# coolbutuseless/zstdlite

Measured on NVIDIA B200. Metric: decompress_GBps_uncompressed, higher is better.
Workload: dtype u8

## Files before the change

### zstdlite_b200/csrc/zl_dec_exec.cuh

```cuda
#pragma once
#include "zl_common.cuh"
#include "zl_dec_entropy.cuh"

#if defined(__CUDACC__)

#define ZL_FULL 0xFFFFFFFFu

ZL_D void zl_warp_copy(u8* dst, const u8* src, u32 n, u32 lane)
{
    if (n < 64) { for (u32 i = lane; i < n; i += 32) dst[i] = src[i]; return; }
    if (((((size_t)dst) ^ ((size_t)src)) & 15) == 0) {
        u32 head = (u32)((16 - (((size_t)dst) & 15)) & 15);
        if (lane < head) dst[lane] = src[lane];
        u32 body = (n - head) >> 4;
        const uint4* s4 = (const uint4*)(src + head);
        uint4* d4 = (uint4*)(dst + head);
        u32 i = lane;
        for (; i + 96 < body; i += 128) {
            const uint4 a = s4[i], b = s4[i + 32], c = s4[i + 64], e = s4[i + 96];
            d4[i] = a; d4[i + 32] = b; d4[i + 64] = c; d4[i + 96] = e;
        }
        for (; i < body; i += 32) d4[i] = s4[i];
        u32 done = head + (body << 4);
        for (u32 i = done + lane; i < n; i += 32) dst[i] = src[i];
        return;
    }
    const u32 head = (u32)((4 - (((size_t)dst) & 3)) & 3);
    if (lane < head) dst[lane] = src[lane];
    const u8* s = src + head;
    u32* d4 = (u32*)(dst + head);
    const u32 words = (n - head) >> 2;
    const u32 sh = (u32)(((size_t)s) & 3) * 8;
    const u32* s4 = (const u32*)(((size_t)s) & ~(size_t)3);
    if (sh == 0) for (u32 i = lane; i < words; i += 32) d4[i] = s4[i];
    else {
        u32 i = lane;
        for (; i + 96 < words; i += 128) {
            const u32 a0 = s4[i], a1 = s4[i + 1], b0 = s4[i + 32], b1 = s4[i + 33], c0 = s4[i + 64], c1 = s4[i + 65], e0 = s4[i + 96], e1 = s4[i + 97];
            d4[i] = __funnelshift_r(a0, a1, sh); d4[i + 32] = __funnelshift_r(b0, b1, sh); d4[i + 64] = __funnelshift_r(c0, c1, sh); d4[i + 96] = __funnelshift_r(e0, e1, sh);
        }
        for (; i < words; i += 32) d4[i] = __funnelshift_r(s4[i], s4[i + 1], sh);
    }
    const u32 done = head + (words << 2);
    if (done + lane < n) dst[done + lane] = src[done + lane];
}

ZL_D void zl_warp_fill(u8* dst, u32 byte, u32 n, u32 lane)
{
    u32 head = (u32)((4 - (((size_t)dst) & 3)) & 3);
    if (head > n) head = n;
    if (lane < head) dst[lane] = (u8)byte;
    u32 body = (n - head) >> 2;
    u32 w = byte * 0x01010101u;
    u32* d4 = (u32*)(dst + head);
    for (u32 i = lane; i < body; i += 32) d4[i] = w;
    u32 done = head + (body << 2);
    for (u32 i = done + lane; i < n; i += 32) dst[i] = (u8)byte;
}

#define ZL_REPT_ID 0x00020100u
ZL_D u32 zl_rept_compose(u32 A, u32 B)
{
    const u32 m = (B >> 7) & 0x00010101u;
    const u32 mm = m * 0xFFu;
    const u32 r = (B & 0x00030303u & ~mm) | (0x00060504u & mm);
    const u32 sel = (r & 0xFu) | ((r >> 4) & 0xF0u) | ((r >> 8) & 0xF00u) | 0x3000u;
    return __byte_perm(A, B, sel) & 0x00FFFFFFu;
}

ZL_D void zl_lane_record(u64 rec, bool valid, const u32* xtab, u32& ll, u32& ml, u32& ob)
{
    ll = 0; ml = 0; ob = 0;
    if (!valid) return;
    if (rec & ZL_REC_B) { ll = (u32)rec & 0xFFFFu; ml = ((u32)rec >> 16) & 0xFFFFu; ob = (u32)(rec >> 32) & 0x7FFFFFFFu; return; }
    const u32 snap = (u32)rec, c = (u32)(rec >> 32);
    const u32 llCode = c & 63u, mlCode = (c >> 6) & 63u, aOF = (c >> 12) & 31u;
    const u32 xl = xtab[llCode], xm = xtab[36 + mlCode];
    const u32 aLL = xl >> 24, aML = xm >> 24;
    ob = (1u << aOF) + zl_shr(snap, 32u - aOF);
    ml = (xm & 0xFFFFFFu) + zl_shr(zl_shl(snap, aOF), 32u - aML);
    ll = (xl & 0xFFFFFFu) + zl_shr(zl_shl(snap, aOF + aML), 32u - aLL);
}
ZL_D u32 zl_rep_idx(u32 ll, u32 ml, u32 ob) { return (ml != 0 && ob >= 1 && ob <= 3) ? ob - 1 + (ll == 0 ? 1u : 0u) : 0u; }
ZL_D u32 zl_rept_of(bool isNew, u32 idx, u32 tag)
{
    if (isNew) return 0x00010000u | 0x80u | tag;
    if (idx == 1) return 0x00020001u;
    if (idx == 2) return 0x00010002u;
    return ZL_REPT_ID;
}
ZL_D u32 zl_rept_scan(u32 T, u32 lane)
{
#pragma unroll
    for (int d = 1; d < 32; d <<= 1) {
        const u32 A = __shfl_up_sync(ZL_FULL, T, d);
        if ((int)lane >= d) T = zl_rept_compose(A, T);
    }
    return T;
}
ZL_D u32 zl_batch_offsets(u32 ll, u32 ml, u32 ob, u32 lane, u32& h0, u32& h1, u32& h2)
{
    const bool isM = ml != 0, isNew = isM && ob >= 4;
    const u32 idx = zl_rep_idx(ll, ml, ob);
    u32 off;
    if (__ballot_sync(ZL_FULL, idx == 3)) {
        off = 0;
        u32 hh[3] = {h0, h1, h2};
        for (u32 l = 0; l < 32; l++) {
            const u32 lll = __shfl_sync(ZL_FULL, ll, l), lml = __shfl_sync(ZL_FULL, ml, l), lob = __shfl_sync(ZL_FULL, ob, l);
            const u32 o = zl_rep_resolve(hh, lll, lml, lob);
            if (l == lane) off = o;
        }
        h0 = hh[0]; h1 = hh[1]; h2 = hh[2];
        return off;
    }
    const u32 fresh = ob - 3;
    const u32 T = zl_rept_scan(zl_rept_of(isNew, idx, lane), lane);
    u32 E = __shfl_up_sync(ZL_FULL, T, 1);
    if (lane == 0) E = ZL_REPT_ID;
    const u32 eb = (E >> (8 * idx)) & 0xFFu;
    const u32 fromLane = __shfl_sync(ZL_FULL, fresh, eb & 31u);
    const u32 fromHist = (eb & 3u) == 0 ? h0 : ((eb & 3u) == 1 ? h1 : h2);
    off = isNew ? fresh : ((eb & 0x80u) ? fromLane : fromHist);
    const u32 Lt = __shfl_sync(ZL_FULL, T, 31);
    const u32 b0 = Lt & 0xFFu, b1 = (Lt >> 8) & 0xFFu, b2 = (Lt >> 16) & 0xFFu;
    const u32 f0 = __shfl_sync(ZL_FULL, fresh, b0 & 31u), f1 = __shfl_sync(ZL_FULL, fresh, b1 & 31u), f2 = __shfl_sync(ZL_FULL, fresh, b2 & 31u);
    const u32 n0 = (b0 & 0x80u) ? f0 : ((b0 & 3u) == 0 ? h0 : ((b0 & 3u) == 1 ? h1 : h2));
    const u32 n1 = (b1 & 0x80u) ? f1 : ((b1 & 3u) == 0 ? h0 : ((b1 & 3u) == 1 ? h1 : h2));
    const u32 n2 = (b2 & 0x80u) ? f2 : ((b2 & 3u) == 0 ? h0 : ((b2 & 3u) == 1 ? h1 : h2));
    h0 = n0; h1 = n1; h2 = n2;
    return off;
}
ZL_D void zl_batch_positions(u32 ll, u32 ml, u32 lane, u32& sl, u32& so, u32& totalL, u32& totalO)
{
    sl = ll; so = ll + ml;
#pragma unroll
    for (int d = 1; d < 32; d <<= 1) {
        u32 a = __shfl_up_sync(ZL_FULL, sl, d), b = __shfl_up_sync(ZL_FULL, so, d);
        if ((int)lane >= d) { sl += a; so += b; }
    }
    totalL = __shfl_sync(ZL_FULL, sl, 31); totalO = __shfl_sync(ZL_FULL, so, 31);
}
ZL_D u32 zl_flat_owner(u32 rs, u32 j)
{
    u32 k = 0;
#pragma unroll
    for (int st = 16; st >= 1; st >>= 1) {
        const u32 v = __shfl_sync(ZL_FULL, rs, (k + st - 1) & 31);
        if (v <= j) k += st;
    }
    return k & 31;
}

#define ZL_SEG_LIT 0x80000000u
#ifndef ZL_XB
#define ZL_XB 4
#endif
#define ZL_XBATCH (32 * ZL_XB)
#define ZL_XROWS (32 * ZL_XB)
struct ZlExecSm {
    uint4 seg[2 * ZL_XBATCH];
    union { u32 fresh[ZL_XBATCH]; uint2 row[ZL_XROWS]; } u;
};
ZL_D uint2 zl_lds64(u32 a) { uint2 v; asm volatile("ld.shared.v2.u32 {%0, %1}, [%2];" : "=r"(v.x), "=r"(v.y) : "r"(a)); return v; }
ZL_D uint4 zl_lds128(u32 a) { uint4 v; asm volatile("ld.shared.v4.u32 {%0, %1, %2, %3}, [%4];" : "=r"(v.x), "=r"(v.y), "=r"(v.z), "=r"(v.w) : "r"(a)); return v; }
ZL_D u32 zl_lds32s(u32 a) { u32 v; asm volatile("ld.shared.u32 %0, [%1];" : "=r"(v) : "r"(a)); return v; }
ZL_D u32 zl_mod_small(u32 k, u32 d, u32 rcpA)
{
    const u32 q = __umulhi(k, zl_lds32s(rcpA + (d << 2)));
    u32 r = k - q * d;
    if (r >= d) r -= d;
    return r;
}
ZL_D const u8* zl_ptr_add(u32 lo, u32 hi, u32 j) { return reinterpret_cast<const u8*>((((u64)hi << 32) | lo) + j); }

ZL_D void zl_batch_offsets4(const u32 (&ll)[ZL_XB], const u32 (&ml)[ZL_XB], const u32 (&ob)[ZL_XB], u32 lane, u32* fresh,
                            u32& h0, u32& h1, u32& h2, u32 (&off)[ZL_XB])
{
    u32 idx[ZL_XB], t[ZL_XB];
    bool minus1 = false;
#pragma unroll
    for (int m = 0; m < ZL_XB; m++) {
        idx[m] = zl_rep_idx(ll[m], ml[m], ob[m]);
        minus1 |= idx[m] == 3;
        t[m] = zl_rept_of(ml[m] != 0 && ob[m] >= 4, idx[m], ZL_XB * lane + (u32)m);
    }
    if (__any_sync(ZL_FULL, minus1)) {
        u32 hh[3] = {h0, h1, h2};
        for (u32 l = 0; l < 32; l++) {
#pragma unroll
            for (int m = 0; m < ZL_XB; m++) {
                const u32 lll = __shfl_sync(ZL_FULL, ll[m], l), lml = __shfl_sync(ZL_FULL, ml[m], l), lob = __shfl_sync(ZL_FULL, ob[m], l);
                const u32 o = zl_rep_resolve(hh, lll, lml, lob);
                if (l == lane) off[m] = o;
            }
        }
        h0 = hh[0]; h1 = hh[1]; h2 = hh[2];
        return;
    }
#if ZL_XB == 4
    *reinterpret_cast<uint4*>(fresh + 4u * lane) = make_uint4(ob[0] - 3u, ob[1] - 3u, ob[2] - 3u, ob[3] - 3u);
    const u32 t01 = zl_rept_compose(t[0], t[1]), t012 = zl_rept_compose(t01, t[2]);
    const u32 T = zl_rept_scan(zl_rept_compose(t012, t[3]), lane);
#else
    *reinterpret_cast<uint2*>(fresh + 2u * lane) = make_uint2(ob[0] - 3u, ob[1] - 3u);
    const u32 t01 = zl_rept_compose(t[0], t[1]);
    const u32 T = zl_rept_scan(t01, lane);
#endif
    u32 E = __shfl_up_sync(ZL_FULL, T, 1);
    if (lane == 0) E = ZL_REPT_ID;
    __syncwarp();
#if ZL_XB == 4
    const u32 e[ZL_XB] = {E, zl_rept_compose(E, t[0]), zl_rept_compose(E, t01), zl_rept_compose(E, t012)};
#else
    const u32 e[ZL_XB] = {E, zl_rept_compose(E, t[0])};
#endif
#pragma unroll
    for (int m = 0; m < ZL_XB; m++) {
        const u32 eb = (e[m] >> (8u * idx[m])) & 0xFFu;
        const u32 fromTag = fresh[eb & (ZL_XBATCH - 1)];
        const u32 fromHist = (eb & 3u) == 0 ? h0 : ((eb & 3u) == 1 ? h1 : h2);
        off[m] = (ml[m] != 0 && ob[m] >= 4) ? ob[m] - 3u : ((eb & 0x80u) ? fromTag : fromHist);
    }
    const u32 Lt = __shfl_sync(ZL_FULL, T, 31);
    const u32 b0 = Lt & 0xFFu, b1 = (Lt >> 8) & 0xFFu, b2 = (Lt >> 16) & 0xFFu;
    const u32 f0 = fresh[b0 & (ZL_XBATCH - 1)], f1 = fresh[b1 & (ZL_XBATCH - 1)], f2 = fresh[b2 & (ZL_XBATCH - 1)];
    const u32 n0 = (b0 & 0x80u) ? f0 : ((b0 & 3u) == 0 ? h0 : ((b0 & 3u) == 1 ? h1 : h2));
    const u32 n1 = (b1 & 0x80u) ? f1 : ((b1 & 3u) == 0 ? h0 : ((b1 & 3u) == 1 ? h1 : h2));
    const u32 n2 = (b2 & 0x80u) ? f2 : ((b2 & 3u) == 0 ? h0 : ((b2 & 3u) == 1 ? h1 : h2));
    h0 = n0; h1 = n1; h2 = n2;
}

template <bool kDict>
ZL_D u32 zl_exec_block(u8* out, u32 op, u32 cap, u32 capErr, const ZlBlockHdr& h, const u8* __restrict__ lit, u32 rleByte, u32 litMode,
                       const u64* __restrict__ recs, const u8* __restrict__ dict, u32 dictSize, u32 (&hist)[3], const u32* xtab, const u32* rcp,
                       ZlExecSm* sm, u32 lane, u32& regen)
{
    const u32 nrec = h.nrec, litSize = h.litSize;
    const u32 leMask = 0xFFFFFFFFu >> (31u - lane);
    const u32 segA = (u32)__cvta_generic_to_shared(sm->seg), rowA = (u32)__cvta_generic_to_shared(sm->u.row), rcpA = (u32)__cvta_generic_to_shared(rcp);
    const bool rleLits = litMode == 1;
    u32 outPos = op, litPos = 0;
    u32 h0 = hist[0], h1 = hist[1], h2 = hist[2];
    auto outPtr = [&](i32 sp) -> const u8* { return (kDict && sp < 0) ? dict + ((i32)dictSize + sp) : out + sp; };
    for (u32 base = 0; base < nrec; base += ZL_XBATCH) {
        const u32 i0 = base + ZL_XB * lane;
        ulonglong2 ra = make_ulonglong2(0ull, 0ull), rb = ra;
        if (i0 < nrec) ra = __ldcs(reinterpret_cast<const ulonglong2*>(recs + i0));
        if (ZL_XB == 4 && i0 + 2 < nrec) rb = __ldcs(reinterpret_cast<const ulonglong2*>(recs + i0 + 2));
        if (i0 + ZL_XBATCH < nrec) asm volatile("prefetch.global.L1 [%0];" ::"l"(recs + i0 + ZL_XBATCH));
        u32 ll[ZL_XB], ml[ZL_XB], ob[ZL_XB], off[ZL_XB];
        zl_lane_record(ra.x, i0 < nrec, xtab, ll[0], ml[0], ob[0]);
        zl_lane_record(ra.y, i0 + 1 < nrec, xtab, ll[1], ml[1], ob[1]);
#if ZL_XB == 4
        zl_lane_record(rb.x, i0 + 2 < nrec, xtab, ll[2], ml[2], ob[2]);
        zl_lane_record(rb.y, i0 + 3 < nrec, xtab, ll[3], ml[3], ob[3]);
#endif
        u32 L = 0, O = 0, nseg = 0;
#pragma unroll
        for (int m = 0; m < ZL_XB; m++) { L += ll[m]; O += ll[m] + ml[m]; nseg += (ll[m] ? 1u : 0u) + (ml[m] ? 1u : 0u); }
        u32 sl = L | (nseg << 23), so = O;
#pragma unroll
        for (int d = 1; d < 32; d <<= 1) {
            const u32 a = __shfl_up_sync(ZL_FULL, sl, d), b = __shfl_up_sync(ZL_FULL, so, d);
            if ((int)lane >= d) { sl += a; so += b; }
        }
        const u32 tot = __shfl_sync(ZL_FULL, sl, 31), totalO = __shfl_sync(ZL_FULL, so, 31);
        const u32 totalL = tot & 0x7FFFFFu;
        if (totalL > litSize - litPos) return ZL_E_corruption_detected;
        if ((outPos - op) + totalO > cap) return capErr;
        zl_batch_offsets4(ll, ml, ob, lane, sm->u.fresh, h0, h1, h2, off);
        const u32 ord0 = (sl >> 23) - nseg;
        u8* const ob8 = out + outPos;
        {
            u32 f = so - O, li = litPos + (sl & 0x7FFFFFu) - L, ord = ord0;
            bool bad = false;
#pragma unroll
            for (int m = 0; m < ZL_XB; m++) {
                if (ll[m]) { const u64 P = (u64)(size_t)lit + li - f; sm->seg[ord++] = make_uint4((u32)P, (u32)(P >> 32), f, ZL_SEG_LIT); }
                f += ll[m]; li += ll[m];
                bad |= ml[m] != 0 && (off[m] == 0 || off[m] > outPos + f + dictSize);
                if (ml[m]) { const u64 P = (u64)(size_t)ob8 - off[m]; sm->seg[ord++] = make_uint4((u32)P, (u32)(P >> 32), f, off[m]); }
                f += ml[m];
            }
            if (__any_sync(ZL_FULL, bad)) return ZL_E_corruption_detected;
        }
        const u32 mis = (u32)((size_t)ob8 & 31u);
        const u32 totalA = totalO + mis;
        u32 segsBefore = 0;
        for (u32 w0 = 0; w0 < totalA; w0 += ZL_XROWS * 32) {
            __syncwarp();
#if ZL_XB == 4
            reinterpret_cast<uint4*>(sm->u.row)[2 * lane] = make_uint4(0u, 0u, 0u, 0u);
            reinterpret_cast<uint4*>(sm->u.row)[2 * lane + 1] = make_uint4(0u, 0u, 0u, 0u);
#else
            reinterpret_cast<uint4*>(sm->u.row)[lane] = make_uint4(0u, 0u, 0u, 0u);
#endif
            __syncwarp();
#pragma unroll
            for (u32 k = 0; k < 2 * ZL_XB; k++) {
                const u32 a = zl_lds32s(segA + (((ord0 + k) & (2 * ZL_XBATCH - 1)) << 4) + 8u) + mis - w0;
                if (k < nseg && a < ZL_XROWS * 32) atomicOr(&sm->u.row[a >> 5].x, 1u << (a & 31u));
            }
            __syncwarp();
            {
#if ZL_XB == 4
                uint4 qa = zl_lds128(rowA + lane * 32u), qb = zl_lds128(rowA + lane * 32u + 16u);
                const u32 c0 = __popc(qa.x), c1 = __popc(qa.z), c2 = __popc(qb.x), c3 = __popc(qb.z);
#else
                uint4 qa = zl_lds128(rowA + lane * 16u);
                const u32 c0 = __popc(qa.x), c1 = __popc(qa.z), c2 = 0, c3 = 0;
#endif
                u32 inc = c0 + c1 + c2 + c3;
#pragma unroll
                for (int d = 1; d < 32; d <<= 1) { const u32 a = __shfl_up_sync(ZL_FULL, inc, d); if ((int)lane >= d) inc += a; }
                const u32 ex = segsBefore + inc - (c0 + c1 + c2 + c3);
                qa.y = ex; qa.w = ex + c0;
#if ZL_XB == 4
                qb.y = ex + c0 + c1; qb.w = ex + c0 + c1 + c2;
                reinterpret_cast<uint4*>(sm->u.row)[2 * lane] = qa;
                reinterpret_cast<uint4*>(sm->u.row)[2 * lane + 1] = qb;
#else
                reinterpret_cast<uint4*>(sm->u.row)[lane] = qa;
#endif
                segsBefore += __shfl_sync(ZL_FULL, inc, 31);
            }
            __syncwarp();
            const u32 wEnd = min(totalA, w0 + ZL_XROWS * 32);
            for (u32 a0 = w0; a0 < wEnd; a0 += 64) {
                const uint4 ri = zl_lds128(rowA + ((a0 - w0) >> 5) * 8u);
                const u32 ja = a0 + lane - mis, jb = ja + 32;
                const u32 d0 = a0 < mis ? lane - (mis - a0) : lane;
                if ((ri.x | ri.z) == 0u && a0 + 64 <= totalA) {
                    const uint4 s = zl_lds128(segA + (((ri.y - 1u) & (2 * ZL_XBATCH - 1)) << 4));
                    u32 va = rleByte, vb = rleByte;
                    if (s.w < 64u) {
                        u32 ta = ja - s.w, tb = jb - s.w;
                        if ((i32)ta >= (i32)s.z) ta = s.z - s.w + zl_mod_small(ja - s.z, s.w, rcpA);
                        if ((i32)tb >= (i32)s.z) tb = s.z - s.w + zl_mod_small(jb - s.z, s.w, rcpA);
                        va = *outPtr((i32)(outPos + ta)); vb = *outPtr((i32)(outPos + tb));
                    } else if (!(s.w == ZL_SEG_LIT && rleLits)) {
                        const u8* pa = zl_ptr_add(s.x, s.y, ja);
                        const u8* pb = zl_ptr_add(s.x, s.y, jb);
                        if (kDict && s.w != ZL_SEG_LIT) { pa = outPtr((i32)(outPos + ja - s.w)); pb = outPtr((i32)(outPos + jb - s.w)); }
                        va = *pa; vb = *pb;
                    }
                    ob8[ja] = (u8)va; ob8[jb] = (u8)vb;
                    __syncwarp();
                    continue;
                }
                const u32 c0 = ri.y + __popc(ri.x & leMask) - 1u, c1 = ri.w + __popc(ri.z & leMask) - 1u;
                const uint4 sa = zl_lds128(segA + ((c0 & (2 * ZL_XBATCH - 1)) << 4)), sb = zl_lds128(segA + ((c1 & (2 * ZL_XBATCH - 1)) << 4));
                const bool aa = ja < totalO, ab = jb < totalO;
                bool na = aa && sa.w <= d0, nb = ab && sb.w <= d0 + 32u;
                const u8* pa = zl_ptr_add(sa.x, sa.y, ja);
                const u8* pb = zl_ptr_add(sb.x, sb.y, jb);
                if (kDict) {
                    if (sa.w != ZL_SEG_LIT) pa = outPtr((i32)(outPos + ja - sa.w));
                    if (sb.w != ZL_SEG_LIT) pb = outPtr((i32)(outPos + jb - sb.w));
                }
                u32 va = rleByte, vb = rleByte;
                if (aa && !na && !(sa.w == ZL_SEG_LIT && rleLits)) va = *pa;
                if (ab && !nb && !(sb.w == ZL_SEG_LIT && rleLits)) vb = *pb;
                if (__any_sync(ZL_FULL, na || nb)) {
                    const u32 j0 = a0 < mis ? 0u : a0 - mis;
                    u32 ta = ja - sa.w, tb = jb - sb.w;
                    if (na && ta >= sa.z) { ta = sa.z - sa.w + zl_mod_small(ja - sa.z, sa.w, rcpA); if ((i32)ta < (i32)j0) { na = false; va = *outPtr((i32)(outPos + ta)); } }
                    if (nb && tb >= sb.z) { tb = sb.z - sb.w + zl_mod_small(jb - sb.z, sb.w, rcpA); if ((i32)tb < (i32)j0) { nb = false; vb = *outPtr((i32)(outPos + tb)); } }
                    const u32 ra_ = ta + mis - a0, rb_ = tb + mis - a0;
                    while (__any_sync(ZL_FULL, na || nb)) {
                        const u32 w = (va & 0xFFu) | (na ? 0u : 0x100u) | ((vb & 0xFFu) << 16) | (nb ? 0u : 0x1000000u);
                        const u32 wa = __shfl_sync(ZL_FULL, w, ra_ & 31u) >> ((ra_ & 32u) >> 1), wb = __shfl_sync(ZL_FULL, w, rb_ & 31u) >> ((rb_ & 32u) >> 1);
                        if (na && (wa & 0x100u)) { va = wa & 0xFFu; na = false; }
                        if (nb && (wb & 0x100u)) { vb = wb & 0xFFu; nb = false; }
                    }
                }
                if (aa) ob8[ja] = (u8)va;
                if (ab) ob8[jb] = (u8)vb;
                __syncwarp();
            }
        }
        outPos += totalO; litPos += totalL;
    }
    const u32 lastLL = litSize - litPos;
    if ((outPos - op) + lastLL > cap) return capErr;
    if (litMode == 1) zl_warp_fill(out + outPos, rleByte, lastLL, lane);
    else zl_warp_copy(out + outPos, lit + litPos, lastLL, lane);
    hist[0] = h0; hist[1] = h1; hist[2] = h2;
    regen = outPos - op + lastLL;
    return 0;
}

#define ZL_P1 0x9E3779B185EBCA87ULL
#define ZL_P2 0xC2B2AE3D27D4EB4FULL
#define ZL_P3 0x165667B19E3779F9ULL
#define ZL_P4 0x85EBCA77C2B2AE63ULL
#define ZL_P5 0x27D4EB2F165667C5ULL
ZL_D u64 zl_rotl64(u64 x, int r) { return (x << r) | (x >> (64 - r)); }
ZL_D u64 zl_xround(u64 acc, u64 in) { return zl_rotl64(acc + in * ZL_P2, 31) * ZL_P1; }
ZL_D u64 zl_xmerge(u64 h, u64 v) { return (h ^ zl_xround(0, v)) * ZL_P1 + ZL_P4; }
ZL_D u64 zl_ld64u(const u8* p)
{
    if ((((size_t)p) & 7) == 0) return *(const u64*)p;
    if ((((size_t)p) & 3) == 0) return (u64)(*(const u32*)p) | ((u64)(*(const u32*)(p + 4)) << 32);
    return zl_rd64(p);
}
ZL_D u64 zl_xxh_seed(u32 q) { return q == 0 ? (ZL_P1 + ZL_P2) : (q == 1 ? ZL_P2 : (q == 2 ? 0ull : (0ull - ZL_P1))); }
ZL_D u64 zl_quad_xxh64_from(const u8* p, u32 len, u64 v, u32 s0, u32 q, u32 qmask, u32 qbase)
{
    u64 h;
    u32 done = 0;
    if (len >= 32) {
        const u32 stripes = len >> 5;
        const u8* pp = p + 8 * q;
        for (u32 s = s0; s < stripes; s++) v = zl_xround(v, zl_ld64u(pp + 32 * s));
        const u64 v1 = __shfl_sync(qmask, v, qbase + 0), v2 = __shfl_sync(qmask, v, qbase + 1);
        const u64 v3 = __shfl_sync(qmask, v, qbase + 2), v4 = __shfl_sync(qmask, v, qbase + 3);
        h = zl_rotl64(v1, 1) + zl_rotl64(v2, 7) + zl_rotl64(v3, 12) + zl_rotl64(v4, 18);
        h = zl_xmerge(h, v1); h = zl_xmerge(h, v2); h = zl_xmerge(h, v3); h = zl_xmerge(h, v4);
        done = stripes << 5;
    } else h = ZL_P5;
    h += (u64)len;
    const u8* t = p + done; u32 r = len - done;
    while (r >= 8) { h ^= zl_xround(0, zl_rd64(t)); h = zl_rotl64(h, 27) * ZL_P1 + ZL_P4; t += 8; r -= 8; }
    if (r >= 4) { h ^= (u64)zl_rd32(t) * ZL_P1; h = zl_rotl64(h, 23) * ZL_P2 + ZL_P3; t += 4; r -= 4; }
    while (r) { h ^= (u64)(*t++) * ZL_P5; h = zl_rotl64(h, 11) * ZL_P1; r--; }
    h ^= h >> 33; h *= ZL_P2; h ^= h >> 29; h *= ZL_P3; h ^= h >> 32;
    return h;
}
ZL_D u64 zl_quad_xxh64(const u8* p, u32 len, u32 q, u32 qmask, u32 qbase) { return zl_quad_xxh64_from(p, len, zl_xxh_seed(q), 0, q, qmask, qbase); }

#define ZL_XXH_CHUNK 2048u
ZL_D u64 zl_warp_xxh64(const u8* p, u32 len, u8 (*buf)[ZL_XXH_CHUNK], u32 lane)
{
    const u32 nchunks = len / ZL_XXH_CHUNK;
    u64 v = zl_xxh_seed(lane & 3);
    if (nchunks) {
        uint4 r[4];
#pragma unroll
        for (int i = 0; i < 4; i++) r[i] = __ldg((const uint4*)p + i * 32 + lane);
        for (u32 c = 0; c < nchunks; c++) {
            uint4* b4 = (uint4*)buf[c & 1];
#pragma unroll
            for (int i = 0; i < 4; i++) b4[i * 32 + lane] = r[i];
            __syncwarp();
            if (c + 1 < nchunks) {
                const uint4* g = (const uint4*)(p + (size_t)(c + 1) * ZL_XXH_CHUNK);
#pragma unroll
                for (int i = 0; i < 4; i++) r[i] = __ldg(g + i * 32 + lane);
            }
            if (lane < 4) {
                const u64* b8 = (const u64*)buf[c & 1] + lane;
#pragma unroll 8
                for (u32 s = 0; s < ZL_XXH_CHUNK / 32; s++) v = zl_xround(v, b8[4 * s]);
            }
        }
        __syncwarp();
    }
    u64 h = 0;
    if (lane < 4) h = zl_quad_xxh64_from(p, len, v, nchunks * (ZL_XXH_CHUNK / 32), lane, 0xFu, 0);
    return __shfl_sync(ZL_FULL, h, 0);
}
#endif
```

### zstdlite_b200/csrc/zl_dec_kernels.cu

```cuda
#include "zl_dec_entropy.cuh"
#include "zl_dec_exec.cuh"
#include "zl_dec_large.cuh"
#include "zl_launch.h"
#include "zl_plan.h"
#include <mutex>
#include <stdlib.h>

__constant__ ZlConstTables c_tables = {
    ZL_LL_BASE_INIT, ZL_ML_BASE_INIT, ZL_LL_BITS_INIT, ZL_ML_BITS_INIT,
    ZL_LL_DEFNORM_INIT, ZL_ML_DEFNORM_INIT, ZL_OF_DEFNORM_INIT};

__global__ void __launch_bounds__(128)
zl_k_index(const ZlFrameDesc* __restrict__ descs, ZlFrameInfo* __restrict__ infos, ZlBlockHdr* hdrArena, ZlUnit* units, u32* unitCount,
           u32 unitCap, u32 nframes, u32 frameBase, const ZlDictDev* dict)
{
    const u32 i = blockIdx.x * blockDim.x + threadIdx.x;
    if (i >= nframes) return;
    const ZlFrameDesc d = descs[i];
    ZlFrameInfo info;
    zl_index_frame(d, info, hdrArena + d.hdrBase, frameBase + i, dict ? dict->dictID : 0u, (dict && dict->hasEntropy) ? 1u : 0u,
                   units, unitCount, unitCap);
    infos[i] = info;
}

__device__ __forceinline__ u32 zl_fetch_units(u32* cursor, u32 lane, u32 count = ZL_QUADS_PER_WARP)
{
    u32 base = 0;
    if (lane == 0) base = atomicAdd(cursor, count);
    return __shfl_sync(0xFFFFFFFFu, base, 0);
}

#ifndef ZL_LIT_RING
#define ZL_LIT_RING 1
#endif
__global__ void __launch_bounds__(32)
zl_k_literals(const ZlFrameDesc* __restrict__ descs, ZlFrameInfo* __restrict__ infos, const ZlBlockHdr* hdrArena,
              u8* litArena, const ZlUnit* __restrict__ units, const u32* __restrict__ unitCount, u32* cursor, const ZlDictDev* dict)
{
    extern __shared__ __align__(16) u8 smraw[];
    ZlLitSm* fs = reinterpret_cast<ZlLitSm*>(smraw);
    const u32 lane = threadIdx.x, quad = lane >> 2, q = lane & 3;
    const u32 qmask = 0xFu << (quad * 4);
    ZlLitSm& f = fs[quad];
    const u32 ring = ZL_LIT_RING ? zl_smem_addr(smraw + ZL_QUADS_PER_WARP * sizeof(ZlLitSm)) + lane * 16u : 0u;
    u16* dictHuf = reinterpret_cast<u16*>(smraw + ZL_QUADS_PER_WARP * sizeof(ZlLitSm) + (ZL_LIT_RING ? ZL_LIT_RING_SLOTS * 32 * 16 : 0));
    if (dict && dict->hasEntropy) {
        const uint4* g = reinterpret_cast<const uint4*>(dict->huf);
        for (u32 i = lane; i < 2048 * 2 / 16; i += 32) reinterpret_cast<uint4*>(dictHuf)[i] = g[i];
        __syncwarp();
    }
    const u32 nunits = *unitCount;
    for (;;) {
        const u32 ubase = zl_fetch_units(cursor, lane);
        if (ubase >= nunits) break;
        const u32 u = ubase + quad;
        if (u < nunits) {
            const ZlUnit un = units[u];
            const ZlFrameDesc d = descs[un.frame];
            const ZlBlockHdr* hdrs = hdrArena + d.hdrBase;
            const u32 litMode = (hdrs[un.block].flags >> 4) & 3;
            if (litMode == 2) {
                u8* lits = (hdrs[un.block].flags & ZL_BLK_DIRECT) ? d.dst + hdrs[un.block].outOff - hdrs[un.block].litOff : litArena + d.litBase;
                const u32 bias = (u32)(((size_t)d.src) & 3);
                const u32* wbase = reinterpret_cast<const u32*>(d.src - bias);
                u32 useDict = 0;
                if (q == 0) zl_lit_unit_head(f, d, hdrs, un.block, wbase, bias, &useDict);
                useDict = __shfl_sync(qmask, useDict, quad * 4);
                __syncwarp(qmask);
                const u32 fill = f.ctl.needHufFill, ns = f.ctl.err ? 0u : f.ctl.nStreams;
                if (useDict) { if (q == 0) f.ctl.hufLog = dict->hufLog; }
                else if (fill && !f.ctl.err) zl_huf_fill(f, q);
                __syncwarp(qmask);
                if (q < ns)
                    f.ctl.sErr[q] = zl_huf_stream(useDict ? dictHuf : f.huf, f.ctl.hufLog, wbase, bias, f.ctl.sBeg[q], f.ctl.sEnd[q],
                                                  lits + f.ctl.sOut[q], f.ctl.sLen[q], ring);
                __syncwarp(qmask);
                if (q == 0) { const u32 e = zl_lit_unit_finish(f); if (e) infos[un.frame].err = e; }
                __syncwarp(qmask);
            }
        }
        __syncwarp();
    }
}

#define ZL_XTAB_BYTES ((ZL_XTAB_WORDS * 4 + 15) & ~15)
#ifndef ZL_SEQ_RING
#define ZL_SEQ_RING 1
#endif
__global__ void __launch_bounds__(32)
zl_k_sequences(const ZlFrameDesc* __restrict__ descs, ZlFrameInfo* __restrict__ infos, ZlBlockHdr* hdrArena,
               u64* recArena, i16* normArena, const ZlUnit* __restrict__ units, const u32* __restrict__ unitCount, u32* cursor,
               const ZlDictDev* dict)
{
    extern __shared__ __align__(16) u8 smraw[];
    u32* xtab = reinterpret_cast<u32*>(smraw);
    ZlSeqSm* fs = reinterpret_cast<ZlSeqSm*>(smraw + ZL_XTAB_BYTES);
    const ZlConstTables& ct = c_tables;
    const u32 lane = threadIdx.x, quad = lane / ZL_SEQ_G, q = lane % ZL_SEQ_G;
    const u32 qmask = (0xFFFFFFFFu >> (32 - ZL_SEQ_G)) << (quad * ZL_SEQ_G);
    for (u32 i = lane; i < ZL_XTAB_WORDS; i += 32)
        xtab[i] = i < 36 ? (c_tables.llBase[i] | ((u32)c_tables.llBits[i] << 24)) : (c_tables.mlBase[i - 36] | ((u32)c_tables.mlBits[i - 36] << 24));
    __syncwarp();
    ZlSeqSm& f = fs[quad];
    const u32 ring = ZL_SEQ_RING ? zl_smem_addr(smraw + ZL_XTAB_BYTES + ZL_SEQ_UNITS * sizeof(ZlSeqSm)) + quad * 16u : 0u;
    i16* norm = normArena + ((size_t)blockIdx.x * ZL_SEQ_UNITS + quad) * (3 * ZL_NORM_STRIDE);
    const u32 nunits = *unitCount;
    const u32 take = (nunits <= 1024u && ZL_SEQ_UNITS > 8u) ? 8u : (u32)ZL_SEQ_UNITS;
    for (;;) {
        const u32 ubase = zl_fetch_units(cursor, lane, take);
        if (ubase >= nunits) break;
        const u32 u = ubase + quad;
        if (quad < take && u < nunits) {
            const ZlUnit un = units[u];
            const ZlFrameDesc d = descs[un.frame];
            ZlBlockHdr* hdrs = hdrArena + d.hdrBase;
            if (hdrs[un.block].nbSeq) {
                const u32 bias = (u32)(((size_t)d.src) & 3);
                const u32* wbase = reinterpret_cast<const u32*>(d.src - bias);
                if (q == 0) zl_seq_head(f, d, hdrs, un.block, ct, norm);
                __syncwarp(qmask);
                const u32 build = f.ctl.err ? 0u : f.ctl.needBuild, useDict = f.ctl.err ? 0u : f.ctl.useDict;
                if (useDict) {
                    if (useDict & 1) { for (u32 i = q; i < 512; i += ZL_SEQ_G) f.fseLL[i] = dict->fseLL[i]; if (q == 0) f.ctl.tlog[0] = dict->tlog[0]; }
                    if (useDict & 2) { for (u32 i = q; i < 256; i += ZL_SEQ_G) f.fseOF[i] = dict->fseOF[i]; if (q == 0) f.ctl.tlog[1] = dict->tlog[1]; }
                    if (useDict & 4) { for (u32 i = q; i < 512; i += ZL_SEQ_G) f.fseML[i] = dict->fseML[i]; if (q == 0) f.ctl.tlog[2] = dict->tlog[2]; }
                }
                if (build) {
#if ZL_SEQ_G >= 3
                    if (q < 3) zl_seq_fse_build(f, q, norm);
#elif ZL_SEQ_G == 2
                    if (q == 0) { zl_seq_fse_build(f, 0, norm); zl_seq_fse_build(f, 1, norm); } else zl_seq_fse_build(f, 2, norm);
#else
                    for (u32 t = 0; t < 3; t++) zl_seq_fse_build(f, t, norm);
#endif
                }
                __syncwarp(qmask);
                if (q == 0) {
                    const u32 nrec = zl_seq_decode(f, recArena + d.recBase + hdrs[un.block].recOff, wbase, bias, ct, xtab, ring);
                    hdrs[un.block].nrec = nrec;
                    if (f.ctl.err) infos[un.frame].err = f.ctl.err;
                }
                __syncwarp(qmask);
            }
        }
        __syncwarp();
    }
}

template <bool kDict>
__global__ void __launch_bounds__(ZL_EXEC_WARPS * 32, ZL_EXEC_MIN_CTAS)
zl_k_execute(const ZlFrameDesc* __restrict__ descs, ZlFrameInfo* __restrict__ infos,
             const ZlBlockHdr* __restrict__ hdrArena, const u64* __restrict__ recArena,
             const u8* __restrict__ litArena, u64* __restrict__ results, u32 nframes, const ZlDictDev* dict)
{
    __shared__ u32 xtab[ZL_XTAB_WORDS];
    __shared__ __align__(16) ZlExecSm execSm[ZL_EXEC_WARPS];
    __shared__ u32 rcp[64];
    for (u32 i = threadIdx.x; i < ZL_XTAB_WORDS; i += ZL_EXEC_WARPS * 32)
        xtab[i] = i < 36 ? (c_tables.llBase[i] | ((u32)c_tables.llBits[i] << 24)) : (c_tables.mlBase[i - 36] | ((u32)c_tables.mlBits[i - 36] << 24));
    if (threadIdx.x < 64) rcp[threadIdx.x] = threadIdx.x ? 0xFFFFFFFFu / threadIdx.x : 0u;
    __syncthreads();
    const u32 lane = threadIdx.x & 31;
    const u32 frame = blockIdx.x * ZL_EXEC_WARPS + (threadIdx.x >> 5);
    if (frame >= nframes) return;
    const ZlFrameInfo info = infos[frame];
    if (info.err) { if (lane == 0) results[frame] = (u64)0 - (u64)info.err; return; }
    const ZlFrameDesc d = descs[frame];
    if (d.large) return;
    const ZlBlockHdr* hdrs = hdrArena + d.hdrBase;
    const u8* dictContent = kDict ? dict->content : nullptr;
    const u32 dictSize = kDict ? dict->contentSize : 0u;
    u32 hist[3] = {1, 4, 8};
    if (kDict && dict->hasEntropy) { hist[0] = dict->rep[0]; hist[1] = dict->rep[1]; hist[2] = dict->rep[2]; }
    u32 op = 0, err = 0;
    for (u32 b = 0; b < info.nblocks && !err; b++) {
        const ZlBlockHdr h = hdrs[b];
        const u32 type = h.flags & 3;
        const u32 room = d.dstCap - op;
        if (type != 2) {
            if (h.regenSize > room) { err = ZL_E_dstSize_tooSmall; break; }
            if (type == 0) zl_warp_copy(d.dst + op, d.src + h.srcOff, h.regenSize, lane);
            else zl_warp_fill(d.dst + op, (h.flags >> 8) & 0xFF, h.regenSize, lane);
            op += h.regenSize;
        } else if (h.flags & ZL_BLK_DIRECT) {
            op += h.litSize;
        } else {
            const u32 litMode = (h.flags >> 4) & 3;
            const u8* lit = litMode == 0 ? d.src + h.srcOff : litArena + d.litBase + h.litOff;
            u32 cap = room, capErr = ZL_E_dstSize_tooSmall, regen = 0;
            if (cap > ZL_BLOCKSIZE_MAX) { cap = ZL_BLOCKSIZE_MAX; capErr = ZL_E_corruption_detected; }
            err = zl_exec_block<kDict>(d.dst, op, cap, capErr, h, lit, (h.flags >> 8) & 0xFF, litMode, recArena + d.recBase + h.recOff,
                                       dictContent, dictSize, hist, xtab, rcp, &execSm[threadIdx.x >> 5], lane, regen);
            op += regen;
        }
        __syncwarp();
    }
    if (!err && info.contentSize != ~0ull && info.contentSize != (u64)op) err = ZL_E_corruption_detected;
    if (lane == 0) {
        results[frame] = err ? (u64)0 - (u64)err : (u64)op;
        infos[frame].err = err; infos[frame].totalOut = op;
    }
}

#define ZL_L_WARPS 4
__device__ __forceinline__ void zl_fill_xtab(u32* xtab, u32 tid, u32 nthreads)
{
    for (u32 i = tid; i < ZL_XTAB_WORDS; i += nthreads)
        xtab[i] = i < 36 ? (c_tables.llBase[i] | ((u32)c_tables.llBits[i] << 24)) : (c_tables.mlBase[i - 36] | ((u32)c_tables.mlBits[i - 36] << 24));
}
__global__ void __launch_bounds__(ZL_L_WARPS * 32)
zl_k_lblock_scan(const u32* __restrict__ largeIdx, const ZlFrameDesc* __restrict__ descs, const ZlFrameInfo* __restrict__ infos,
                 const ZlBlockHdr* __restrict__ hdrArena, const u64* __restrict__ recArena, ZlLChunk* lcArena)
{
    __shared__ u32 xtab[ZL_XTAB_WORDS];
    zl_fill_xtab(xtab, threadIdx.x, ZL_L_WARPS * 32);
    __syncthreads();
    const u32 frame = largeIdx[blockIdx.y], c = blockIdx.z * ZL_L_WARPS + (threadIdx.x >> 5), lane = threadIdx.x & 31;
    const ZlFrameInfo info = infos[frame];
    if (info.err) return;
    const ZlFrameDesc d = descs[frame];
    ZlLChunk* lc = lcArena + ((d.recBase >> ZL_LCHUNK_LOG) + d.hdrBase);
    for (u32 b = blockIdx.x; b < info.nblocks; b += gridDim.x) {
        const ZlBlockHdr h = hdrArena[d.hdrBase + b];
        if ((h.flags & 3) != 2 || !h.nrec || c >= zl_lchunks(h.nrec)) continue;
        const u32 r0 = c << ZL_LCHUNK_LOG, r1 = min(h.nrec, r0 + ZL_LCHUNK_RECS);
        zl_lchunk_scan(recArena + d.recBase + h.recOff, r0, r1, xtab, lane, lc[zl_lchunk_index(h.recOff, b) + c]);
    }
}
__global__ void __launch_bounds__(128)
zl_k_lblock_compose(const u32* __restrict__ largeIdx, const ZlFrameDesc* __restrict__ descs, const ZlFrameInfo* __restrict__ infos,
                    const ZlBlockHdr* __restrict__ hdrArena, ZlLBlock* lbArena, ZlLChunk* lcArena, u32 spread)
{
    const u32 frame = largeIdx[blockIdx.y];
    const ZlFrameInfo info = infos[frame];
    if (info.err) return;
    const ZlFrameDesc d = descs[frame];
    ZlLChunk* lc = lcArena + ((d.recBase >> ZL_LCHUNK_LOG) + d.hdrBase);
    for (u32 b = blockIdx.x * 128 + threadIdx.x; b < info.nblocks; b += gridDim.x * 128) {
        const ZlBlockHdr h = hdrArena[d.hdrBase + b];
        ZlLChunk* C = lc + zl_lchunk_index(h.recOff, b);
        if (spread) zl_lblock_spread(h, lbArena[d.hdrBase + b], C);
        else zl_lblock_compose(h, C, lbArena[d.hdrBase + b]);
    }
}
__global__ void __launch_bounds__(32)
zl_k_lframe_prefix(const u32* __restrict__ largeIdx, const ZlFrameDesc* __restrict__ descs, ZlFrameInfo* __restrict__ infos,
                   const ZlBlockHdr* __restrict__ hdrArena, ZlLBlock* lbArena, const ZlDictDev* dict)
{
    const u32 frame = largeIdx[blockIdx.x];
    if (threadIdx.x != 0) return;
    const ZlFrameInfo info = infos[frame];
    if (info.err) return;
    const ZlFrameDesc d = descs[frame];
    u32 r0 = 1, r1 = 4, r2 = 8, total = 0;
    if (dict && dict->hasEntropy) { r0 = dict->rep[0]; r1 = dict->rep[1]; r2 = dict->rep[2]; }
    const u32 err = zl_lframe_prefix(d, info, hdrArena + d.hdrBase, lbArena + d.hdrBase, r0, r1, r2, &total);
    infos[frame].err = err; infos[frame].totalOut = total;
}
template <bool kDict>
__global__ void __launch_bounds__(ZL_L_WARPS * 32)
zl_k_lblock_emit(const u32* __restrict__ largeIdx, const ZlFrameDesc* __restrict__ descs, ZlFrameInfo* __restrict__ infos,
                 const ZlBlockHdr* __restrict__ hdrArena, const u64* __restrict__ recArena, const u8* __restrict__ litArena,
                 const ZlLBlock* __restrict__ lbArena, const ZlLChunk* __restrict__ lcArena, u32* parentArena, const ZlDictDev* dict)
{
    __shared__ u32 xtab[ZL_XTAB_WORDS];
    zl_fill_xtab(xtab, threadIdx.x, ZL_L_WARPS * 32);
    __syncthreads();
    const u32 frame = largeIdx[blockIdx.y], c = blockIdx.z * ZL_L_WARPS + (threadIdx.x >> 5), lane = threadIdx.x & 31;
    const ZlFrameInfo info = infos[frame];
    if (info.err) return;
    const ZlFrameDesc d = descs[frame];
    const ZlLChunk* lc = lcArena + ((d.recBase >> ZL_LCHUNK_LOG) + d.hdrBase);
    for (u32 b = blockIdx.x; b < info.nblocks; b += gridDim.x) {
        const ZlBlockHdr h = hdrArena[d.hdrBase + b];
        const bool comp = (h.flags & 3) == 2;
        const u32 nch = comp ? zl_lchunks(h.nrec) : 1u;
        if (c >= nch) continue;
        const u32 litMode = (h.flags >> 4) & 3;
        const u8* lit = litMode == 0 ? d.src + h.srcOff : litArena + d.litBase + h.litOff;
        const u32 r0 = c << ZL_LCHUNK_LOG, r1 = comp ? min(h.nrec, r0 + ZL_LCHUNK_RECS) : 0u;
        const u32 err = zl_lchunk_emit<kDict>(d.dst, parentArena + d.parBase, d, h, lbArena[d.hdrBase + b], lc[comp ? zl_lchunk_index(h.recOff, b) + c : 0u], r0, r1,
                                              c + 1 == nch, lit, recArena + d.recBase + h.recOff, kDict ? dict->content : nullptr,
                                              kDict ? dict->contentSize : 0u, xtab, lane);
        if (err && lane == 0) infos[frame].err = err;
    }
}
__global__ void __launch_bounds__(256)
zl_k_ljump(const u32* __restrict__ largeIdx, const ZlFrameDesc* __restrict__ descs, const ZlFrameInfo* __restrict__ infos, u32* parentArena,
           u32* remain, u32 pass)
{
    if (pass > 1 && remain[pass - 1] == 0) return;
    const u32 frame = largeIdx[blockIdx.y];
    const ZlFrameInfo info = infos[frame];
    if (info.err) return;
    const ZlFrameDesc d = descs[frame];
    u32* parent = parentArena + d.parBase;
    u8* out = d.dst;
    u32 open = 0;
    for (u32 p = blockIdx.x * 256 + threadIdx.x; p < info.totalOut; p += gridDim.x * 256) {
        const u32 v = parent[p];
        if (v >= ZL_PAR_DONE) continue;
        const u32 pv = __ldcg(parent + v);
        if (pv >= ZL_PAR_DONE) {
            if ((pv & 0xFFu) < pass) { out[p] = __ldcg(out + v); parent[p] = ZL_PAR_DONE | pass; }
            else open++;
        } else {
            const u32 pv2 = __ldcg(parent + pv);
            if (pv2 >= ZL_PAR_DONE) {
                if ((pv2 & 0xFFu) < pass) { out[p] = __ldcg(out + pv); parent[p] = ZL_PAR_DONE | pass; }
                else { parent[p] = pv; open++; }
            } else { parent[p] = pv2; open++; }
        }
    }
// ... 256 lines not shown
```

Measured before the change: 220.0.

## Widen sequence execution to 4 bytes per lane with 32-bit global loads/stores

The warp execution loop now covers 128 output bytes per iteration, with each lane producing a 4-byte word instead of two single bytes. Uniform segments use funnel-shifted word loads from literals, history or the dictionary, plus one 32-bit store. Mixed spans resolve up to four bytes per lane, using per-byte segment lookups and shuffle-based dependency resolution. The short-offset threshold rises from 64 to 128 and the reciprocal table is enlarged to match, which adds register pressure and more complex divergent paths.

Measured after the change: 180.7, median of 6. 17.8% lower.

```diff
diff --git a/zstdlite_b200/csrc/zl_dec_exec.cuh b/zstdlite_b200/csrc/zl_dec_exec.cuh
--- a/zstdlite_b200/csrc/zl_dec_exec.cuh
+++ b/zstdlite_b200/csrc/zl_dec_exec.cuh
@@ -165,6 +165,7 @@
 ZL_D uint2 zl_lds64(u32 a) { uint2 v; asm volatile("ld.shared.v2.u32 {%0, %1}, [%2];" : "=r"(v.x), "=r"(v.y) : "r"(a)); return v; }
 ZL_D uint4 zl_lds128(u32 a) { uint4 v; asm volatile("ld.shared.v4.u32 {%0, %1, %2, %3}, [%4];" : "=r"(v.x), "=r"(v.y), "=r"(v.z), "=r"(v.w) : "r"(a)); return v; }
 ZL_D u32 zl_lds32s(u32 a) { u32 v; asm volatile("ld.shared.u32 %0, [%1];" : "=r"(v) : "r"(a)); return v; }
+#define ZL_RCP_N 128
 ZL_D u32 zl_mod_small(u32 k, u32 d, u32 rcpA)
 {
     const u32 q = __umulhi(k, zl_lds32s(rcpA + (d << 2)));
@@ -173,6 +174,27 @@
     return r;
 }
 ZL_D const u8* zl_ptr_add(u32 lo, u32 hi, u32 j) { return reinterpret_cast<const u8*>((((u64)hi << 32) | lo) + j); }
+ZL_D u32 zl_ldg8(const u8* p) { __builtin_assume(__isGlobal(p)); return *p; }
+ZL_D u32 zl_ldg32(const u8* p) { __builtin_assume(__isGlobal(p)); return *reinterpret_cast<const u32*>(p); }
+ZL_D void zl_stg8(u8* p, u32 v) { __builtin_assume(__isGlobal(p)); *p = (u8)v; }
+ZL_D void zl_stg32(u8* p, u32 v) { __builtin_assume(__isGlobal(p)); *reinterpret_cast<u32*>(p) = v; }
+ZL_D u32 zl_ldg_word(const u8* p)
+{
+    const u8* q = reinterpret_cast<const u8*>((size_t)p & ~(size_t)3);
+    const u32 sh = (u32)((size_t)p & 3) * 8u;
+    const u32 lo = zl_ldg32(q);
+    return sh ? __funnelshift_r(lo, zl_ldg32(q + 4), sh) : lo;
+}
+template <bool kDict>
+ZL_D u32 zl_out_word(const u8* out, i32 sp, const u8* dict, u32 dictSize)
+{
+    if (!kDict || sp >= 0) return zl_ldg_word(out + sp);
+    if (sp <= -4) return zl_ldg_word(dict + ((i32)dictSize + sp));
+    u32 v = 0;
+#pragma unroll
+    for (i32 k = 0; k < 4; k++) v |= zl_ldg8(sp + k < 0 ? dict + ((i32)dictSize + sp + k) : out + (sp + k)) << (8 * k);
+    return v;
+}
 
 ZL_D void zl_batch_offsets4(const u32 (&ll)[ZL_XB], const u32 (&ml)[ZL_XB], const u32 (&ob)[ZL_XB], u32 lane, u32* fresh,
                             u32& h0, u32& h1, u32& h2, u32 (&off)[ZL_XB])
@@ -237,7 +259,6 @@
                        ZlExecSm* sm, u32 lane, u32& regen)
 {
     const u32 nrec = h.nrec, litSize = h.litSize;
-    const u32 leMask = 0xFFFFFFFFu >> (31u - lane);
     const u32 segA = (u32)__cvta_generic_to_shared(sm->seg), rowA = (u32)__cvta_generic_to_shared(sm->u.row), rcpA = (u32)__cvta_generic_to_shared(rcp);
     const bool rleLits = litMode == 1;
     u32 outPos = op, litPos = 0;
@@ -285,7 +306,7 @@
             }
             if (__any_sync(ZL_FULL, bad)) return ZL_E_corruption_detected;
         }
-        const u32 mis = (u32)((size_t)ob8 & 31u);
+        const u32 mis = (u32)((size_t)ob8 & 127u);
         const u32 totalA = totalO + mis;
         u32 segsBefore = 0;
         for (u32 w0 = 0; w0 < totalA; w0 += ZL_XROWS * 32) {
@@ -327,56 +348,94 @@
             }
             __syncwarp();
             const u32 wEnd = min(totalA, w0 + ZL_XROWS * 32);
-            for (u32 a0 = w0; a0 < wEnd; a0 += 64) {
-                const uint4 ri = zl_lds128(rowA + ((a0 - w0) >> 5) * 8u);
-                const u32 ja = a0 + lane - mis, jb = ja + 32;
-                const u32 d0 = a0 < mis ? lane - (mis - a0) : lane;
-                if ((ri.x | ri.z) == 0u && a0 + 64 <= totalA) {
+            for (u32 a0 = w0; a0 < wEnd; a0 += 128) {
+                const uint2 ri = zl_lds64(rowA + ((((a0 - w0) >> 5) + (lane >> 3)) << 3));
+                const u32 J0 = a0 - mis;
+                const u32 j = J0 + 4u * lane;
+                u32 v;
+                if (!__any_sync(ZL_FULL, ri.x != 0u) && a0 + 128 <= totalA) {
                     const uint4 s = zl_lds128(segA + (((ri.y - 1u) & (2 * ZL_XBATCH - 1)) << 4));
-                    u32 va = rleByte, vb = rleByte;
-                    if (s.w < 64u) {
-                        u32 ta = ja - s.w, tb = jb - s.w;
-                        if ((i32)ta >= (i32)s.z) ta = s.z - s.w + zl_mod_small(ja - s.z, s.w, rcpA);
-                        if ((i32)tb >= (i32)s.z) tb = s.z - s.w + zl_mod_small(jb - s.z, s.w, rcpA);
-                        va = *outPtr((i32)(outPos + ta)); vb = *outPtr((i32)(outPos + tb));
-                    } else if (!(s.w == ZL_SEG_LIT && rleLits)) {
-                        const u8* pa = zl_ptr_add(s.x, s.y, ja);
-                        const u8* pb = zl_ptr_add(s.x, s.y, jb);
-                        if (kDict && s.w != ZL_SEG_LIT) { pa = outPtr((i32)(outPos + ja - s.w)); pb = outPtr((i32)(outPos + jb - s.w)); }
-                        va = *pa; vb = *pb;
+                    if (s.w == ZL_SEG_LIT) v = rleLits ? rleByte * 0x01010101u : zl_ldg_word(zl_ptr_add(s.x, s.y, j));
+                    else if (s.w >= 128u) v = zl_out_word<kDict>(out, (i32)(outPos + j - s.w), dict, dictSize);
+                    else {
+                        const u32 m0 = zl_mod_small(j - s.z, s.w, rcpA);
+                        const i32 sp = (i32)(outPos + s.z - s.w);
+                        if (m0 + 4u <= s.w) v = zl_out_word<kDict>(out, sp + (i32)m0, dict, dictSize);
+                        else {
+                            v = 0;
+#pragma unroll
+                            for (u32 k = 0; k < 4; k++) {
+                                u32 m = m0 + k;
+                                if (m >= s.w) m -= s.w;
+                                if (m >= s.w) m -= s.w;
+                                if (m >= s.w) m -= s.w;
+                                v |= zl_ldg8(outPtr(sp + (i32)m)) << (8 * k);
+                            }
+                        }
                     }
-                    ob8[ja] = (u8)va; ob8[jb] = (u8)vb;
+                    zl_stg32(ob8 + j, v);
                     __syncwarp();
                     continue;
                 }
-                const u32 c0 = ri.y + __popc(ri.x & leMask) - 1u, c1 = ri.w + __popc(ri.z & leMask) - 1u;
-                const uint4 sa = zl_lds128(segA + ((c0 & (2 * ZL_XBATCH - 1)) << 4)), sb = zl_lds128(segA + ((c1 & (2 * ZL_XBATCH - 1)) << 4));
-                const bool aa = ja < totalO, ab = jb < totalO;
-                bool na = aa && sa.w <= d0, nb = ab && sb.w <= d0 + 32u;
-                const u8* pa = zl_ptr_add(sa.x, sa.y, ja);
-                const u8* pb = zl_ptr_add(sb.x, sb.y, jb);
-                if (kDict) {
-                    if (sa.w != ZL_SEG_LIT) pa = outPtr((i32)(outPos + ja - sa.w));
-                    if (sb.w != ZL_SEG_LIT) pb = outPtr((i32)(outPos + jb - sb.w));
-                }
-                u32 va = rleByte, vb = rleByte;
-                if (aa && !na && !(sa.w == ZL_SEG_LIT && rleLits)) va = *pa;
-                if (ab && !nb && !(sb.w == ZL_SEG_LIT && rleLits)) vb = *pb;
-                if (__any_sync(ZL_FULL, na || nb)) {
-                    const u32 j0 = a0 < mis ? 0u : a0 - mis;
-                    u32 ta = ja - sa.w, tb = jb - sb.w;
-                    if (na && ta >= sa.z) { ta = sa.z - sa.w + zl_mod_small(ja - sa.z, sa.w, rcpA); if ((i32)ta < (i32)j0) { na = false; va = *outPtr((i32)(outPos + ta)); } }
-                    if (nb && tb >= sb.z) { tb = sb.z - sb.w + zl_mod_small(jb - sb.z, sb.w, rcpA); if ((i32)tb < (i32)j0) { nb = false; vb = *outPtr((i32)(outPos + tb)); } }
-                    const u32 ra_ = ta + mis - a0, rb_ = tb + mis - a0;
-                    while (__any_sync(ZL_FULL, na || nb)) {
-                        const u32 w = (va & 0xFFu) | (na ? 0u : 0x100u) | ((vb & 0xFFu) << 16) | (nb ? 0u : 0x1000000u);
-                        const u32 wa = __shfl_sync(ZL_FULL, w, ra_ & 31u) >> ((ra_ & 32u) >> 1), wb = __shfl_sync(ZL_FULL, w, rb_ & 31u) >> ((rb_ & 32u) >> 1);
-                        if (na && (wa & 0x100u)) { va = wa & 0xFFu; na = false; }
-                        if (nb && (wb & 0x100u)) { vb = wb & 0xFFu; nb = false; }
+                const u32 b0 = (lane & 7u) << 2;
+                const u32 jlo = (i32)J0 < 0 ? 0u : J0;
+                const uint4 s = zl_lds128(segA + (((ri.y + __popc(ri.x & (0xFFFFFFFFu >> (31u - b0))) - 1u) & (2 * ZL_XBATCH - 1)) << 4));
+                const bool full = j < totalO && totalO - j >= 4u;
+                const u8* pk[4];
+                u32 ldm = 0, unres = 0, rp = 0;
+                v = 0;
+                {
+                    uint4 sk = s;
+                    u32 cprev = 0;
+#pragma unroll
+                    for (u32 k = 0; k < 4; k++) {
+                        const u32 jk = j + k;
+                        if (k) {
+                            const u32 ck = __popc(ri.x & (0xFFFFFFFFu >> (31u - b0 - k)));
+                            if (ck != cprev) sk = zl_lds128(segA + (((ri.y + ck - 1u) & (2 * ZL_XBATCH - 1)) << 4));
+                            cprev = ck;
+                        } else cprev = __popc(ri.x & (0xFFFFFFFFu >> (31u - b0)));
+                        pk[k] = (kDict && sk.w != ZL_SEG_LIT) ? outPtr((i32)(outPos + jk - sk.w)) : zl_ptr_add(sk.x, sk.y, jk);
+                        if (jk >= totalO) continue;
+                        if (sk.w == ZL_SEG_LIT && rleLits) v |= rleByte << (8 * k);
+                        else if (sk.w > jk - jlo) ldm |= 1u << k;
+                        else {
+                            u32 t = jk - sk.w;
+                            if (t >= sk.z) t = sk.z - sk.w + zl_mod_small(jk - sk.z, sk.w, rcpA);
+                            if ((i32)t >= (i32)jlo) { unres |= 1u << k; rp |= (t - J0) << (8 * k); }
+                            else { pk[k] = outPtr((i32)(outPos + t)); ldm |= 1u << k; }
+                        }
                     }
                 }
-                if (aa) ob8[ja] = (u8)va;
-                if (ab) ob8[jb] = (u8)vb;
+                const bool word = full && ldm == 0xFu && ((ri.x >> b0) & 0xEu) == 0u && pk[3] == pk[0] + 3;
+                const u8* q = reinterpret_cast<const u8*>((size_t)pk[0] & ~(size_t)3);
+                const u32 sh = (u32)((size_t)pk[0] & 3) * 8u;
+                u32 lo = 0, hi = 0, x0 = 0, x1 = 0, x2 = 0, x3 = 0;
+                if (word) lo = zl_ldg32(q);
+                if (word && sh) hi = zl_ldg32(q + 4);
+                if (!word && (ldm & 1u)) x0 = zl_ldg8(pk[0]);
+                if (!word && (ldm & 2u)) x1 = zl_ldg8(pk[1]);
+                if (!word && (ldm & 4u)) x2 = zl_ldg8(pk[2]);
+                if (!word && (ldm & 8u)) x3 = zl_ldg8(pk[3]);
+                v |= word ? __funnelshift_r(lo, hi, sh) : (x0 | (x1 << 8) | (x2 << 16) | (x3 << 24));
+                if (__any_sync(ZL_FULL, unres != 0u)) {
+                    do {
+#pragma unroll
+                        for (u32 k = 0; k < 4; k++) {
+                            const u32 r = (rp >> (8 * k)) & 0x7Fu;
+                            const u32 wv = __shfl_sync(ZL_FULL, v, r >> 2), wu = __shfl_sync(ZL_FULL, unres, r >> 2);
+                            if (((unres >> k) & 1u) && !((wu >> (r & 3u)) & 1u)) {
+                                v |= ((wv >> (8 * (r & 3u))) & 0xFFu) << (8 * k);
+                                unres &= ~(1u << k);
+                            }
+                        }
+                    } while (__any_sync(ZL_FULL, unres != 0u));
+                }
+                if (full) zl_stg32(ob8 + j, v);
+                else {
+#pragma unroll
+                    for (u32 k = 0; k < 4; k++) if (j + k < totalO) zl_stg8(ob8 + (j + k), v >> (8 * k));
+                }
                 __syncwarp();
             }
         }
diff --git a/zstdlite_b200/csrc/zl_dec_kernels.cu b/zstdlite_b200/csrc/zl_dec_kernels.cu
--- a/zstdlite_b200/csrc/zl_dec_kernels.cu
+++ b/zstdlite_b200/csrc/zl_dec_kernels.cu
@@ -155,10 +155,10 @@
 {
     __shared__ u32 xtab[ZL_XTAB_WORDS];
     __shared__ __align__(16) ZlExecSm execSm[ZL_EXEC_WARPS];
-    __shared__ u32 rcp[64];
+    __shared__ u32 rcp[ZL_RCP_N];
     for (u32 i = threadIdx.x; i < ZL_XTAB_WORDS; i += ZL_EXEC_WARPS * 32)
         xtab[i] = i < 36 ? (c_tables.llBase[i] | ((u32)c_tables.llBits[i] << 24)) : (c_tables.mlBase[i - 36] | ((u32)c_tables.mlBits[i - 36] << 24));
-    if (threadIdx.x < 64) rcp[threadIdx.x] = threadIdx.x ? 0xFFFFFFFFu / threadIdx.x : 0u;
+    for (u32 i = threadIdx.x; i < ZL_RCP_N; i += ZL_EXEC_WARPS * 32) rcp[i] = i ? 0xFFFFFFFFu / i : 0u;
     __syncthreads();
     const u32 lane = threadIdx.x & 31;
     const u32 frame = blockIdx.x * ZL_EXEC_WARPS + (threadIdx.x >> 5);
```
